# Desperodoo/distributed_multi_agent_reinforcement_learning

Hardware: AMD Instinct MI355X
Metric: env-steps/sec (whole node), pursuit-evasion 8-agent 4096-env (higher is better)
Workload: dtype f64 environment / f32 policy (f32 matrix products evaluated from exact 3-way bf16 operand splits, f32 accumulation and storage)

## Files before the change

### distributed_multi_agent_reinforcement_learning_amd/csrc/mappo_split.hip

```cpp
#include <hip/hip_runtime.h>
#include <stdint.h>
#include <string.h>

#include "mappo_ops.h"
#include "sb_gemm.hpp"
#include "sb_gru_seq.hpp"

extern "C" {

static int sb_gemm_any(int64_t R, int32_t N, int32_t K, const float *X, int64_t ldx, const float *W, int64_t ldw, const float *bias, int32_t relu,
                       const float *addend, int64_t lda, float *Y, int64_t ldy, uint8_t *ybits, int64_t ldyb, void *stream) {
    if (R < 0 || !X || !W || !Y || ldx < K || ldw < K || ldy < N || (addend && lda < N)) return MO_ERR_BAD_ARG;
    if ((ldx & 3) || (ldw & 3) || (ldy & 3) || (lda & 3) || ((uintptr_t)X & 15) || ((uintptr_t)W & 15) || ((uintptr_t)Y & 15) || ((uintptr_t)addend & 15) ||
        ((uintptr_t)bias & 15))
        return MO_ERR_BAD_ARG;
    if (R == 0) return 0;
    hipStream_t st = (hipStream_t)stream;
    if (N == 128 && K == 128) return launch_sb_gemm_best<4, 1>(R, X, ldx, W, ldw, bias, addend, lda, Y, ldy, relu, st, ybits, ldyb);
    if (N == 128 && K == 256) return launch_sb_gemm_best<8, 1>(R, X, ldx, W, ldw, bias, addend, lda, Y, ldy, relu, st, ybits, ldyb);
    if (ybits) return MO_ERR_BAD_ARG;
    if (N == 128 && K == 384) return launch_sb_gemm_best<12, 1>(R, X, ldx, W, ldw, bias, addend, lda, Y, ldy, relu, st);
    if (N == 256 && K == 128) return launch_sb_gemm_best<4, 2>(R, X, ldx, W, ldw, bias, addend, lda, Y, ldy, relu, st);
    if (N == 384 && K == 128) return launch_sb_gemm_best<4, 3>(R, X, ldx, W, ldw, bias, addend, lda, Y, ldy, relu, st);
    return MO_ERR_BAD_ARG;
}

int sb_gemm(int64_t R, int32_t N, int32_t K, const float *X, int64_t ldx, const float *W, int64_t ldw, const float *bias, int32_t relu,
            const float *addend, int64_t lda, float *Y, int64_t ldy, void *stream) {
    return sb_gemm_any(R, N, K, X, ldx, W, ldw, bias, relu, addend, lda, Y, ldy, nullptr, 0, stream);
}

int sb_gemm_signs(int64_t R, int32_t N, int32_t K, const float *X, int64_t ldx, const float *W, int64_t ldw, const float *bias, int32_t relu,
                  const float *addend, int64_t lda, float *Y, int64_t ldy, uint8_t *y_sign_bits, int64_t ld_bytes, void *stream) {
    if (!y_sign_bits || ld_bytes < N / 8) return MO_ERR_BAD_ARG;
    return sb_gemm_any(R, N, K, X, ldx, W, ldw, bias, relu, addend, lda, Y, ldy, y_sign_bits, ld_bytes, stream);
}

int64_t sb_gemm_masked_workspace(int32_t N) { return N > 0 ? (int64_t)1024 * N * 4 : 0; }

int sb_gemm_masked(int64_t R, int32_t N, int32_t K, const float *X, int64_t ldx, const float *W, int64_t ldw, const float *M, int64_t ldm,
                   int32_t mask_cols, float *Y, int64_t ldy, float *colsum, void *workspace, void *stream) {
    if (R < 0 || !X || !W || !M || !Y || !colsum || !workspace || ldx < K || ldw < K || ldy < N || ldm < N) return MO_ERR_BAD_ARG;
    if (mask_cols < 0 || mask_cols > N || (mask_cols & 127)) return MO_ERR_BAD_ARG;
    if ((ldx & 3) || (ldw & 3) || (ldy & 3) || (ldm & 3) || ((uintptr_t)X & 15) || ((uintptr_t)W & 15) || ((uintptr_t)Y & 15) || ((uintptr_t)M & 15) ||
        ((uintptr_t)colsum & 15) || ((uintptr_t)workspace & 15))
        return MO_ERR_BAD_ARG;
    hipStream_t st = (hipStream_t)stream;
    if (R == 0) return (int)hipMemsetAsync(colsum, 0, (size_t)N * 4, st);
    int dev = 0, cus = 256;
    if (hipGetDevice(&dev) == hipSuccess && hipDeviceGetAttribute(&cus, hipDeviceAttributeMultiprocessorCount, dev) != hipSuccess) cus = 256;
    if (cus > 512) return MO_ERR_BAD_ARG;
    float *part = (float *)workspace;
// ... 60 lines not shown
```

### distributed_multi_agent_reinforcement_learning_amd/csrc/sb_gemm.hpp

```cpp
#pragma once
#include <mutex>

#include "sb_common.hpp"

#ifndef SBG_ABLATE
#define SBG_ABLATE 0
#endif

template <int KC, int NT, int OPT = 3>
__global__ __launch_bounds__(512) void k_sb_gemm_n128(int64_t R, const float *__restrict__ X, int64_t ldx, const float *__restrict__ W, int64_t ldw,
                                                      const float *__restrict__ bias, const float *addend, int64_t lda, float *Y, int64_t ldy, int relu,
                                                      int mask_tiles, float *__restrict__ colsum_part, uint8_t *__restrict__ ybits = nullptr, int64_t ldyb = 0) {
    extern __shared__ uint4 sbg_tile[];
    constexpr int IMG = 3 * KC * 2 * 64, UPW = KC / 4;
    const int tid = threadIdx.x, w = tid >> 6, l = tid & 63, i = l & 15, gq = l >> 4;
    uint4 wg[NT][KC][3];
    float4 b4[NT];
#pragma unroll
    for (int t = 0; t < NT; t++) {
        const float *rw = W + (size_t)(16 * (w + 8 * t) + i) * ldw + 8 * gq;
#pragma unroll
        for (int c = 0; c < KC; c++) sb_split8(*(const float4 *)(rw + 32 * c), *(const float4 *)(rw + 32 * c + 4), wg[t][c]);
        b4[t] = !(OPT & 4) && bias ? *(const float4 *)(bias + 16 * (w + 8 * t) + 4 * gq) : make_float4(0.f, 0.f, 0.f, 0.f);
    }
    const int64_t n_it = (R + 31) / 32;
    float4 pf[UPW][2];
    auto fetch = [&](int64_t it) {
#pragma unroll
        for (int n = 0; n < UPW; n++) {
            const int blk = w * UPW + n, c = blk >> 1, rt = blk & 1;
            const int64_t row = it * 32 + rt * 16 + i;
            pf[n][0] = pf[n][1] = make_float4(0.f, 0.f, 0.f, 0.f);
            if (row < R) {
                const float *src = X + row * ldx + 32 * c + 8 * gq;
                if constexpr (SBG_ABLATE & 4) {
                    pf[n][0] = pf[n][1] = make_float4((float)row * 1e-6f, 0.5f, -0.25f, (float)c);
                } else {
                    pf[n][0] = *(const float4 *)src;
                    pf[n][1] = *(const float4 *)(src + 4);
                }
            }
        }
    };
    auto stage = [&](uint4 *img) {
#pragma unroll
        for (int n = 0; n < UPW; n++) {
            const int blk = w * UPW + n;
            uint4 p_[3];
            sb_split8(pf[n][0], pf[n][1], p_);
#pragma unroll
            for (int p = 0; p < 3; p++) img[(p * KC * 2 + blk) * 64 + l] = p_[p];
        }
    };
    int64_t it = blockIdx.x;
    if (it < n_it) { fetch(it); stage(sbg_tile); }
    if (it + gridDim.x < n_it) fetch(it + gridDim.x);
    lds_barrier();
    int cur = 0;
    float4 cs[NT];
#pragma unroll
    for (int t = 0; t < NT; t++) cs[t] = make_float4(0.f, 0.f, 0.f, 0.f);
    for (; it < n_it; it += gridDim.x) {
        const uint4 *tb = sbg_tile + cur * IMG + l;
        f32x4 acc[NT][2];
        float4 a4[NT][2];
        if ((OPT & 1) && addend) {
#pragma unroll
            for (int rt = 0; rt < 2; rt++) {
                const int64_t row = it * 32 + rt * 16 + i;
#pragma unroll
                for (int t = 0; t < NT; t++)
                    a4[t][rt] = row < R ? *(const float4 *)(addend + row * lda + 16 * (w + 8 * t) + 4 * gq) : make_float4(0.f, 0.f, 0.f, 0.f);
            }
        }
        auto next_tile = [&]() {
// ... 38 lines not shown
            if constexpr (AHEAD) __builtin_amdgcn_sched_barrier(0);
        }
        if (!(OPT & 2) || w >= 4) next_tile();
        unsigned mb[NT][2];
        if constexpr ((OPT & 4) && (OPT & 16)) {
            __builtin_amdgcn_sched_barrier(0);
            const uint8_t *bits = (const uint8_t *)addend;
#pragma unroll
            for (int rt = 0; rt < 2; rt++) {
                const int64_t row = it * 32 + rt * 16 + i;
#pragma unroll
                for (int t = 0; t < NT; t++)
                    mb[t][rt] = row < R && t < mask_tiles ? (unsigned)bits[row * lda + 2 * (w + 8 * t) + (gq >> 1)] >> ((gq & 1) * 4) : 15u;
            }
        } else if constexpr ((OPT & 4) && !(OPT & 1)) {
            __builtin_amdgcn_sched_barrier(0);
#pragma unroll
            for (int rt = 0; rt < 2; rt++) {
                const int64_t row = it * 32 + rt * 16 + i;
#pragma unroll
                for (int t = 0; t < NT; t++)
                    a4[t][rt] = row < R && t < mask_tiles ? *(const float4 *)(addend + row * lda + 16 * (w + 8 * t) + 4 * gq) : make_float4(1.f, 1.f, 1.f, 1.f);
            }
        }
#pragma unroll
        for (int rt = 0; rt < 2; rt++) {
            const int64_t row = it * 32 + rt * 16 + i;
            if (row < R) {
#pragma unroll
                for (int t = 0; t < NT; t++) {
                    const int col = 16 * (w + 8 * t) + 4 * gq;
                    float4 v;
                    if constexpr (OPT & 4) {
                        v = make_float4(acc[t][rt][0], acc[t][rt][1], acc[t][rt][2], acc[t][rt][3]);
                        if constexpr (OPT & 16) {
                            const unsigned m = mb[t][rt];
                            v.x = (m & 1u) ? v.x : 0.f; v.y = (m & 2u) ? v.y : 0.f; v.z = (m & 4u) ? v.z : 0.f; v.w = (m & 8u) ? v.w : 0.f;
                        } else if (t < mask_tiles) {
                            v.x = a4[t][rt].x > 0.f ? v.x : 0.f; v.y = a4[t][rt].y > 0.f ? v.y : 0.f;
                            v.z = a4[t][rt].z > 0.f ? v.z : 0.f; v.w = a4[t][rt].w > 0.f ? v.w : 0.f;
                        }
                        cs[t].x += v.x; cs[t].y += v.y; cs[t].z += v.z; cs[t].w += v.w;
                    } else {
                        v = make_float4(acc[t][rt][0] + b4[t].x, acc[t][rt][1] + b4[t].y, acc[t][rt][2] + b4[t].z, acc[t][rt][3] + b4[t].w);
                        if (addend) {
                            if (!(OPT & 1)) a4[t][rt] = *(const float4 *)(addend + row * lda + col);
                            v.x += a4[t][rt].x; v.y += a4[t][rt].y; v.z += a4[t][rt].z; v.w += a4[t][rt].w;
                        }
                        if (relu) { v.x = fmaxf(v.x, 0.f); v.y = fmaxf(v.y, 0.f); v.z = fmaxf(v.z, 0.f); v.w = fmaxf(v.w, 0.f); }
                        if constexpr (OPT & 8) {
                            const unsigned nib = (unsigned)(v.x > 0.f) | ((unsigned)(v.y > 0.f) << 1) | ((unsigned)(v.z > 0.f) << 2) | ((unsigned)(v.w > 0.f) << 3);
                            const unsigned other = (unsigned)__shfl_xor((int)nib, 16);
                            if (!(gq & 1)) ybits[row * ldyb + 2 * (w + 8 * t) + (gq >> 1)] = (uint8_t)(nib | (other << 4));
                        }
                    }
                    if constexpr (SBG_ABLATE & 2) { if (v.x == 12345.678f) *(float4 *)(Y + row * ldy + col) = v; }
                    else *(float4 *)(Y + row * ldy + col) = v;
                }
            }
        }
        lds_barrier();
        cur ^= 1;
    }
    if constexpr (OPT & 4) {
#pragma unroll
        for (int t = 0; t < NT; t++) {
#pragma unroll
            for (int m = 1; m < 16; m <<= 1) {
                cs[t].x += __shfl_xor(cs[t].x, m); cs[t].y += __shfl_xor(cs[t].y, m);
                cs[t].z += __shfl_xor(cs[t].z, m); cs[t].w += __shfl_xor(cs[t].w, m);
            }
            if (i == 0) *(float4 *)(colsum_part + (size_t)blockIdx.x * (128 * NT) + 16 * (w + 8 * t) + 4 * gq) = cs[t];
        }
    }
}

__global__ void k_sb_colsum_reduce(int n_parts, int F, const float *__restrict__ parts, float *__restrict__ out) {
    const int f = blockIdx.x * blockDim.x + threadIdx.x;
    if (f >= F) return;
    float a0 = 0.f, a1 = 0.f, a2 = 0.f, a3 = 0.f;
    int p = 0;
    for (; p + 4 <= n_parts; p += 4) {
        a0 += parts[(size_t)p * F + f]; a1 += parts[(size_t)(p + 1) * F + f];
        a2 += parts[(size_t)(p + 2) * F + f]; a3 += parts[(size_t)(p + 3) * F + f];
    }
    for (; p < n_parts; p++) a0 += parts[(size_t)p * F + f];
    out[f] = (a0 + a1) + (a2 + a3);
}

static int g_sbg_wgs_per_cu = 0;

template <int KC, int NT, int OPT>
int launch_sb_gemm(int64_t R, const float *X, int64_t ldx, const float *W, int64_t ldw, const float *bias, const float *addend, int64_t lda,
                   float *Y, int64_t ldy, int relu, hipStream_t st, int mask_tiles = 0, float *colsum_part = nullptr, float *colsum = nullptr,
                   uint8_t *ybits = nullptr, int64_t ldyb = 0) {
    constexpr int lds = 2 * 3 * KC * 2 * 64 * 16;
    static std::once_flag once;
    static hipError_t attr_rc = hipSuccess;
    std::call_once(once, [] { attr_rc = hipFuncSetAttribute((const void *)k_sb_gemm_n128<KC, NT, OPT>, hipFuncAttributeMaxDynamicSharedMemorySize, lds); });
    if (attr_rc != hipSuccess) return (int)attr_rc;
    int dev = 0, cus = 256;
    if (hipGetDevice(&dev) == hipSuccess && hipDeviceGetAttribute(&cus, hipDeviceAttributeMultiprocessorCount, dev) != hipSuccess) cus = 256;
    const int64_t n_it = (R + 31) / 32;
    const int wpc = g_sbg_wgs_per_cu ? g_sbg_wgs_per_cu : (KC * NT == 4 && R >= 131072 ? 2 : 1);
    const int grid = n_it < (int64_t)cus * wpc ? (int)n_it : cus * wpc;
    hipLaunchKernelGGL((k_sb_gemm_n128<KC, NT, OPT>), dim3(grid), dim3(512), lds, st, R, X, ldx, W, ldw, bias, addend, lda, Y, ldy, relu, mask_tiles,
                       colsum_part, ybits, ldyb);
    if constexpr (OPT & 4) hipLaunchKernelGGL(k_sb_colsum_reduce, dim3((128 * NT + 127) / 128), dim3(128), 0, st, grid, 128 * NT, colsum_part, colsum);
    return (int)hipGetLastError();
}

constexpr int SBG_MASK_OPT_256 = 6, SBG_MASK_OPT_384 = 4, SBG_MASK_OPT_K384 = 6;

template <int KC, int NT>
int launch_sb_gemm_best(int64_t R, const float *X, int64_t ldx, const float *W, int64_t ldw, const float *bias, const float *addend, int64_t lda,
                        float *Y, int64_t ldy, int relu, hipStream_t st, uint8_t *ybits = nullptr, int64_t ldyb = 0) {
    constexpr int PLAIN = (KC == 4 && NT == 1) ? 0 : 2;
    constexpr int ADD = KC == 12 ? 2 : (KC == 8 ? 3 : (NT == 3 ? 0 : 1));
    if constexpr (NT == 1 && KC <= 8) if (ybits) {
        if (addend) return launch_sb_gemm<KC, NT, ADD | 8>(R, X, ldx, W, ldw, bias, addend, lda, Y, ldy, relu, st, 0, nullptr, nullptr, ybits, ldyb);
        if constexpr (KC == 4 && NT == 1) if (R >= 786432) return launch_sb_gemm<4, 1, 10>(R, X, ldx, W, ldw, bias, addend, lda, Y, ldy, relu, st, 0, nullptr, nullptr, ybits, ldyb);
        return launch_sb_gemm<KC, NT, PLAIN | 8>(R, X, ldx, W, ldw, bias, addend, lda, Y, ldy, relu, st, 0, nullptr, nullptr, ybits, ldyb);
    }
    if (addend) return launch_sb_gemm<KC, NT, ADD>(R, X, ldx, W, ldw, bias, addend, lda, Y, ldy, relu, st);
    if constexpr (KC == 4 && NT == 1) if (R >= 786432) return launch_sb_gemm<4, 1, 2>(R, X, ldx, W, ldw, bias, addend, lda, Y, ldy, relu, st);
    return launch_sb_gemm<KC, NT, PLAIN>(R, X, ldx, W, ldw, bias, addend, lda, Y, ldy, relu, st);
}
```

### distributed_multi_agent_reinforcement_learning_amd/model.py

```python
import torch
import torch.nn as nn
import torch.nn.functional as F
from torch.nn.utils import spectral_norm
from torch.nn.utils.spectral_norm import SpectralNorm

from . import ops


class HeadLinear(nn.Linear):

    def forward(self, x):
        return ops.linear_skinny(x, self.weight, self.bias)


def _ortho_linear(n_in, n_out, cls=nn.Linear):
    layer = cls(n_in, n_out)
    for name, param in layer.named_parameters():
        if "bias" in name:
            nn.init.constant_(param, 0)
        elif "weight" in name:
            nn.init.orthogonal_(param, gain=1.0)
    return layer


# ... 26 lines not shown
        self.AGG_layers["AGG_vertex_0"] = _make_linear(E, E, is_sn)
        for k in range(self.depth):
            self.AGG_layers[f"AGG_fcra_{k}"] = _make_linear(E, E, is_sn)

    def encoder(self, p, e, o, adj_p, adj_e, adj_o, is_critic, o_kvalid=None, q_div=1, out=None, e_ref=None):
        M = self.MSG_layers
        m3 = ops.msg_agg3(p, e, o, adj_p, adj_e, adj_o, M[0].weight, M[0].bias, M[1].weight, M[1].bias, M[2].weight, M[2].bias,
                          is_critic, o_kvalid, q_div, e_ref)
        return self._after_messages(p, m3, out)

    def _after_messages(self, p, m3, out=None):
        R, P = p.shape[0], p.shape[1]
        E, ind = self.embedding_dim, self.input_dim
        agg0 = self.AGG_layers["AGG_vertex_0"]
        link = ops.ReluLink()
        emb = ops.linear(m3, agg0.weight, agg0.bias, relu=True, y_link=link)
        Ws = self.semantic_layer.weight
        p2, e2 = p.reshape(R * P, ind), emb.reshape(R * P, 3 * E)
        if out is not None:
            o2 = out.view(R * P, E)
            torch.addmm(self.semantic_layer.bias, p2, Ws[:, :ind].t(), out=o2)
            h0 = o2.addmm_(e2, Ws[:, ind:].t())
        else:
            h0 = ops.linear(e2, Ws[:, ind:], ops.linear_skinny(p2, Ws[:, :ind], self.semantic_layer.bias), consume_addend=True, x_link=link)
        return h0.reshape(R, P, E)

    def encoder_pair_train(self, p, e, o, adj_p, adj_e, adj_o, q_div=1, e_ref=None):
        M = self.MSG_layers
        m3a, m3c = ops.msg_agg3_pair_train(p, e, o, adj_p, adj_e, adj_o, M[0].weight, M[0].bias, M[1].weight, M[1].bias, M[2].weight, M[2].bias,
                                           q_div, e_ref)
        return self._after_messages(p, m3a), self._after_messages(p, m3c)

    def fcra(self, h0, hist, adj_p, is_critic, out=None):
        if self.depth == 0:
            return h0
        h, carry = h0, None
        for k in range(self.depth):
            aggk, fk = self.AGG_layers[f"AGG_fcra_{k}"], self.FCRA_layers[k]
            nb = ops.fcra_mean(z_critic=hist[k]) if is_critic else ops.fcra_mean(z_actor=hist[k], adj=adj_p)
            last = k == self.depth - 1
            h, carry = ops.fcra_hop(nb, h, carry, aggk.weight, aggk.bias, fk.weight, fk.bias, last, out if last else None)
        h.relu_link = carry[1]
        return h

    def forward(self, p, e, o, adj_p, adj_e, adj_o, hist, is_critic, o_kvalid=None, q_div=1, out=None, e_ref=None):
        h0 = self.encoder(p, e, o, adj_p, adj_e, adj_o, is_critic, o_kvalid, q_div, out if self.depth == 0 else None, e_ref)
        return self.fcra(h0, hist, adj_p, is_critic, out)

    def forward_pair(self, p, e, o, adj_p, adj_e, adj_o, hist_a, hist_c, o_kvalid=None, q_div=1, out=None, e_ref=None):
        R, P = p.shape[0], p.shape[1]
        E, ind = self.embedding_dim, self.input_dim
        M = self.MSG_layers
        Ws = self.semantic_layer.weight
        d = self.depth
        cats = [torch.empty((2, R, P, 2 * E), dtype=p.dtype, device=p.device) for _ in range(d)]
        if d:
            h0 = cats[0][..., E:]
        else:
            h0 = out if out is not None else torch.empty((2, R, P, E), dtype=p.dtype, device=p.device)
        h0_2d = ops.block2d(h0)
        fused_pos = ind == 4
        m3 = ops.msg_agg3_pair(p, e, o, adj_p, adj_e, adj_o, M[0].weight, M[0].bias, M[1].weight, M[1].bias, M[2].weight, M[2].bias,
                               o_kvalid, q_div, pos=(Ws[:, :ind], self.semantic_layer.bias, h0) if fused_pos else None, e_ref=e_ref)
        agg0 = self.AGG_layers["AGG_vertex_0"]
        m3_2d = m3.view(-1, E)
        if ops.split_linear_ok(m3_2d, agg0.weight):
            emb = ops.split_linear(m3_2d, agg0.weight, agg0.bias, relu=True).view(m3.shape)
        else:
            emb = ops.linear(m3, agg0.weight, agg0.bias, relu=True)
        if not fused_pos:
            torch.addmm(self.semantic_layer.bias, p.reshape(R * P, ind), Ws[:, :ind].t(), out=h0_2d[:R * P])
            h0_2d[R * P:].copy_(h0_2d[:R * P])
        emb_2d, Wse = emb.view(2 * R * P, 3 * E), Ws[:, ind:]
        if ops.split_linear_ok(emb_2d, Wse, h0_2d, h0_2d):
            ops.split_linear(emb_2d, Wse, None, False, out=h0_2d, addend=h0_2d)
        elif d:
            ops.gemm_nt(emb_2d, Wse, None, False, out=h0_2d, addend=h0_2d)
        else:
            h0_2d.addmm_(emb_2d, Wse.t())
        if d == 0:
            return h0
        h = h0
        zas, zcs = [], []
        for k in range(d):
            aggk = self.AGG_layers[f"AGG_fcra_{k}"]

            def lin(z, W=aggk.weight):
                if z.is_contiguous() and ops.split_linear_ok(z.view(-1, E), W):
                    return ops.split_linear(z.view(-1, E), W).view(z.shape)
                return ops.linear(z, W)
            za = lin(hist_a[k])
            zcs.append(za if hist_c[k] is hist_a[k] or hist_c[k].data_ptr() == hist_a[k].data_ptr() else lin(hist_c[k]))
            zas.append(za)
        if d <= 4 and all(z.is_contiguous() for z in zas + zcs) and adj_p.dtype == torch.float32:
            ops.fcra_mean_pair_multi(zas, zcs, adj_p, [self.AGG_layers[f"AGG_fcra_{k}"].bias for k in range(d)], [cats[k][..., :E] for k in range(d)])
        else:
            for k in range(d):
# ... 233 lines not shown
```

### distributed_multi_agent_reinforcement_learning_amd/ops.py

```python
import ctypes as C
import os

import torch
import torch.nn.functional as F

from . import build as _build

ADJ_TENSOR, ADJ_ONES, ADJ_VALID, ADJ_BITS = 0, 1, 2, 3
EXPORTS = ("dhgn_msg_agg_fwd", "dhgn_msg_agg3_fwd", "dhgn_msg_agg_bwd", "dhgn_msg_agg_bwd_workspace", "dhgn_msg_agg_ones_sorted_ok", "dhgn_msg_agg_ones_sorted_fwd",
           "dhgn_msg_agg_ones_sorted_bwd", "dhgn_msg_agg_ones_sorted_workspace", "gae_advnorm", "gae_advnorm_workspace", "categorical_sample",
           "categorical_sample_counter",
           "gru_gates_fwd", "gru_gates_bwd", "gru_cell_fwd", "gru_cell_fwd_multi", "gru_cell_split_fwd_multi", "sb_gemm_n128", "sb_gemm", "gru_seq_fwd", "gru_seq_fwd_multi", "gru_seq_split_fwd_multi", "gru_seq_split_bwd_multi", "gru_seq_save_elems", "gru_seq_bwd", "gru_seq_bwd_multi", "gru_seq_bwd_workspace", "wgrad_tn", "wgrad_tn_workspace", "wgrad_split_tn", "wgrad_split_tn2", "wgrad_split_workspace", "rollout_record", "ppo_loss_fwd_bwd", "ppo_loss_prob_fwd_bwd", "ppo_loss_workspace",
           "gauss_head_sample", "ppo_loss_gauss_fwd_bwd", "ppo_loss_gauss_workspace", "gauss_head_sample_ex", "ppo_loss_gauss_ex_fwd_bwd",
           "ppo_loss_gauss_ex_workspace", "gae_advnorm_vn", "gae_advnorm_vn_workspace", "value_norm_update", "value_norm_targets",
           "ppo_loss_fwd_bwd_diag", "ppo_loss_prob_fwd_bwd_diag", "ppo_loss_gauss_fwd_bwd_diag", "ppo_loss_gauss_ex_fwd_bwd_diag",
           "ppo_loss_diag_workspace", "ppo_loss_gauss_diag_workspace", "ppo_ratio", "ppo_diag_rows_host", "fused_adam_workspace",
           "fused_adam_grid", "fused_adam_norm", "fused_adam_step", "fused_adam_advance_host", "fused_adam_rows_host", "bc_loss_workspace",
           "bc_loss_gauss_fwd_bwd", "bc_loss_gauss_ex_fwd_bwd", "bc_loss_cat_fwd_bwd", "e3d_bc_select", "n2n_bc_select", "mappo_ops_error_string")

_lib = None


def lib_path():
    return _build.lib_path("libmappo_ops.so")


def load_library():
    global _lib
    if _lib is None:
        path = lib_path()
        if not os.path.exists(path):
            raise RuntimeError(f"{path} is missing: build it with __graft_entry__.build() (hipcc --offload-arch=gfx950); "
                               "the fused MAPPO ops have no fallback")
        L = C.CDLL(path)
        vp, i32, i64, f32, f64 = C.c_void_p, C.c_int32, C.c_int64, C.c_float, C.c_double
# ... 11 lines not shown
        L.dhgn_msg_agg_ones_sorted_workspace.argtypes = [i32, i32, i32, i32, i32, vp, vp, vp]
        L.dhgn_msg_agg_ones_sorted_workspace.restype = i64
        L.dhgn_msg_agg_ones_sorted_fwd.argtypes = [i32, i32, i32, i32, vp, i64, vp, i64, i32, vp, vp, vp, i64, vp, vp, vp]
        L.dhgn_msg_agg_ones_sorted_bwd.argtypes = [i32, i32, i32, i32, vp, i64, i32, vp, i64, vp, vp, vp, vp, vp, vp]
        L.gae_advnorm.argtypes = [i32, i32, i32, vp, vp, vp, f32, f32, i32, vp, vp, vp, vp]
        L.gae_advnorm_workspace.restype = i64
        L.gae_advnorm_vn.argtypes = [i32, i32, i32, vp, vp, vp, vp, vp, f32, f32, i32, vp, vp, vp, vp, vp]
        L.gae_advnorm_vn_workspace.restype = i64
        L.value_norm_update.argtypes = [vp, vp, C.c_double, vp]
        L.value_norm_targets.argtypes = [i64, vp, vp, vp, vp, vp]
        L.categorical_sample.argtypes = [i32, i32, vp, C.c_uint64, C.c_uint64, i32, vp, vp, vp]
        L.categorical_sample_counter.argtypes = [i32, i32, vp, C.c_uint64, vp, i32, vp, vp, vp]
        L.head_linear.argtypes = [i32, i32, i32, vp, vp, vp, vp, vp]
        L.head_sample.argtypes = [i32, i32, i32, vp, vp, vp, C.c_uint64, vp, vp, i32, vp, vp, vp]
        L.gru_gates_fwd.argtypes = [i32, i32, vp, vp, vp, vp, vp, vp, vp]
        L.gru_gates_bwd.argtypes = [i32, i32, vp, vp, vp, vp, vp, vp, vp, vp]
        L.gru_cell_fwd.argtypes = [i32, i32, vp, vp, vp, vp, vp, vp, vp, vp]
        L.gru_seq_fwd.argtypes = [i32, i32, i32, vp, vp, vp, vp, vp, vp, i32, vp]
        L.gru_seq_bwd.argtypes = [i32, i32, i32, vp, vp, vp, vp, vp, vp, vp, vp, vp, vp, vp, i32, vp, vp]
        L.gru_cell_fwd_multi.argtypes = [i32, vp, i32, i32, vp]
        L.gru_cell_split_fwd_multi.argtypes = [i32, vp, i32, i32, vp]
        L.sb_gemm_n128.argtypes = [i64, i32, vp, i64, vp, i64, vp, i32, vp, i64, vp, i64, vp]
        L.sb_gemm.argtypes = [i64, i32, i32, vp, i64, vp, i64, vp, i32, vp, i64, vp, i64, vp]
        L.gru_seq_fwd_multi.argtypes = [i32, vp, i32, i32, i32, i32, vp]
        L.gru_seq_bwd_multi.argtypes = [i32, vp, i32, i32, i32, i32, vp]
        L.gru_seq_split_fwd_multi.argtypes = [i32, vp, i32, i32, i32, i32, vp]
        L.gru_seq_split_bwd_multi.argtypes = [i32, vp, i32, i32, i32, i32, vp]
        L.gru_seq_save_elems.argtypes = [i32, i32]
        L.gru_seq_save_elems.restype = i64
        L.gru_seq_bwd_workspace.argtypes = [i32]
        L.gru_seq_bwd_workspace.restype = i64
        L.wgrad_tn_workspace.argtypes = [i32, i32]
        L.wgrad_tn_workspace.restype = i64
        L.wgrad_tn.argtypes = [i64, i32, i32, vp, i64, vp, i64, vp, i32, vp, vp]
        L.wgrad_split_workspace.restype = i64
        L.wgrad_split_workspace.argtypes = [i32, i32]
        L.wgrad_split_tn.argtypes = [i64, i32, i32, vp, i64, vp, i64, vp, i32, vp, vp]
        L.wgrad_split_tn2.argtypes = [i64, i32, i32, i32, vp, i64, vp, i64, vp, i64, vp, i32, vp, vp]
        L.fcra_neighbour_mean.argtypes = [i32, i32, i32, i32, vp, i64, i64, vp, i64, i64, vp, i64, vp, i32, vp, vp, i64, vp]
        L.fcra_neighbour_mean_multi.argtypes = [i32, vp, i32, i32, i32, i32, i64, i64, i64, i64, vp, i64, i32, i64, vp]
        L.sb_gemm_signs.argtypes = [i64, i32, i32, vp, i64, vp, i64, vp, i32, vp, i64, vp, i64, vp, i64, vp]
        L.sb_gemm_masked_bits.argtypes = [i64, i32, i32, vp, i64, vp, i64, vp, i64, i32, vp, i64, vp, vp, vp]
        L.sb_gemm_masked_workspace.argtypes = [i32]
        L.sb_gemm_masked_workspace.restype = i64
        L.sb_gemm_masked.argtypes = [i64, i32, i32, vp, i64, vp, i64, vp, i64, i32, vp, i64, vp, vp, vp]
        L.relu_bwd_colsum_workspace.argtypes = [i32]
# ... 1552 lines not shown
    MATMUL_MODE, WGRAD_MODE, PROJ_MODE, CELL_MODE, SEQ_MODE = modes


def set_matmul_mode(mode):
    global MATMUL_MODE, WGRAD_MODE, PROJ_MODE, SEQ_MODE
    set_cell_mode(mode)
    MATMUL_MODE = WGRAD_MODE = PROJ_MODE = SEQ_MODE = mode


SPLIT_LINEAR_SHAPES = {(128, 128), (128, 256), (128, 384), (256, 128), (384, 128)}
UPDATE_SPLIT_SHAPES = SPLIT_LINEAR_SHAPES


def split_linear_ok(x, W, out=None, addend=None, mode=None, shapes=None):
    if ((CELL_MODE if mode is None else mode) != "split_bf16" or torch.is_grad_enabled() or not x.is_cuda
            or tuple(W.shape) not in (SPLIT_LINEAR_SHAPES if shapes is None else shapes)):
        return False
    for t in (x, W) + ((out,) if out is not None else ()) + ((addend,) if addend is not None else ()):
        if t.dtype != torch.float32 or t.dim() != 2 or t.stride(1) != 1 or t.stride(0) % 4 or t.data_ptr() % 16:
            return False
    return x.shape[1] == W.shape[1]


def split_linear(x, W, bias=None, relu=False, out=None, addend=None, sign_bits=None):
    L = load_library()
    R, K = x.shape
    N = W.shape[0]
    W = W.detach()
    if out is None:
        out = torch.empty((R, N), dtype=torch.float32, device=x.device)
    b = bias.detach() if bias is not None else None
    if sign_bits is not None:
        assert sign_bits.dtype == torch.uint8 and sign_bits.shape == (R, N // 8) and sign_bits.stride(1) == 1 and sign_bits_ok(N, K)
        _check(L.sb_gemm_signs(R, N, K, _ptr(x), x.stride(0), _ptr(W), W.stride(0), _ptr(b), int(bool(relu)), _ptr(addend),
                               addend.stride(0) if addend is not None else 0, _ptr(out), out.stride(0), _ptr(sign_bits), sign_bits.stride(0), _stream()),
               "sb_gemm_signs")
        return out
    _check(L.sb_gemm(R, N, K, _ptr(x), x.stride(0), _ptr(W), W.stride(0), _ptr(b), int(bool(relu)), _ptr(addend),
                     addend.stride(0) if addend is not None else 0, _ptr(out), out.stride(0), _stream()), "sb_gemm")
    return out


def sign_bits_ok(N, K):
    return RELU_LINK and RELU_BITS and N == 128 and K in (128, 256)


PROJ_MODE = os.environ.get("MAPPO_PROJ", MATMUL_MODE)


def gru_input_projection(x2, w_ih, b_ih):
    if x2.stride(-1) == 1 and split_linear_ok(x2, w_ih, mode=PROJ_MODE, shapes=UPDATE_SPLIT_SHAPES):
        return split_linear(x2, w_ih, b_ih)
    return torch.addmm(b_ih, x2, w_ih.t())


def gru_step_multi(xs, hiddens, modules, hiddens_out=None):
    n = len(xs)
    B = xs[0].shape[0]
    outs_h = hiddens if hiddens_out is None else hiddens_out
    ok = (not torch.is_grad_enabled() and n <= 4 and B >= FUSED_CELL_MIN_ROWS and all(x.shape == (B, 128) and x.is_cuda for x in xs)
          and all(h.is_contiguous() and h.shape[1:] == (B, 128) for h in list(hiddens) + list(outs_h))
          and all(m.num_layers == modules[0].num_layers and m.weight_hh_l0.shape == (384, 128) and m.weight_ih_l0.shape == (384, 128) for m in modules))
    if not ok:
# ... 203 lines not shown
```

### include/mappo_ops.h

```cpp
#ifndef MAPPO_OPS_H
#define MAPPO_OPS_H
#include <stdint.h>

#ifdef __cplusplus
extern "C" {
#endif

#define MO_ERR_BAD_ARG 20001

enum { MO_ADJ_TENSOR = 0,
       MO_ADJ_ONES = 1,
       MO_ADJ_VALID = 2,
       MO_ADJ_BITS = 3 };
#define MO_ADJ_ROW_WORDS(K) (((((K) + 31) >> 5) + 3) & ~3)

int dhgn_msg_agg_fwd(int32_t R, int32_t P, int32_t K, int32_t E, int32_t din, const float *p, int64_t p_row_stride,
                     const float *q, int64_t q_row_stride, int32_t q_div, const float *e, int64_t e_row_stride, const void *adj,
                     int64_t adj_row_stride, int32_t adj_mode, const int32_t *kvalid, const float *W, const float *b,
                     float *out, int64_t out_stride , void *stream);

typedef struct mo_msg_rel {
    int32_t K, din, q_div, adj_mode;
    const float *q; int64_t q_rs;
    const float *e; int64_t e_rs;
// ... 79 lines not shown
    void *workspace;
    int32_t B, pad0;
} mo_gru_seq_bwd_net;
int gru_seq_fwd_multi(int32_t n_nets, const mo_gru_seq_net *nets, int32_t T, int32_t B, int32_t H, int32_t gi_agents, void *stream);
int gru_seq_bwd_multi(int32_t n_nets, const mo_gru_seq_bwd_net *nets, int32_t T, int32_t B, int32_t H, int32_t gi_agents, void *stream);
int gru_seq_split_fwd_multi(int32_t n_nets, const mo_gru_seq_net *nets, int32_t T, int32_t B, int32_t H, int32_t gi_agents, void *stream);
int gru_seq_split_bwd_multi(int32_t n_nets, const mo_gru_seq_bwd_net *nets, int32_t T, int32_t B, int32_t H, int32_t gi_agents, void *stream);
int gru_seq_fwd(int32_t T, int32_t B, int32_t H, const float *gi, const float *w_hh, const float *b_hh, const float *h0, float *out,
                float *save, int32_t gi_agents, void *stream);
int64_t gru_seq_bwd_workspace(int32_t B);
int gru_seq_bwd(int32_t T, int32_t B, int32_t H, const float *dout, const float *save, const float *out, const float *h0,
                const float *w_hh, float *dgi, float *dgh, float *dnr, float *dh0, float *db_ih, float *db_hh, int32_t gi_agents,
                void *workspace, void *stream);

int gru_cell_fwd(int32_t B, int32_t H, const float *x, const float *h_prev, const float *w_ih, const float *w_hh, const float *b_ih,
                 const float *b_hh, float *h_out, void *stream);
typedef struct mo_gru_cell_net { const float *x, *h_prev, *w_ih, *w_hh, *b_ih, *b_hh; float *h_out; } mo_gru_cell_net;
int gru_cell_fwd_multi(int32_t n_nets, const mo_gru_cell_net *nets, int32_t B, int32_t H, void *stream);
int gru_cell_split_fwd_multi(int32_t n_nets, const mo_gru_cell_net *nets, int32_t B, int32_t H, void *stream);
int sb_gemm_n128(int64_t R, int32_t K, const float *X, int64_t ldx, const float *W, int64_t ldw, const float *bias, int32_t relu, const float *C,
                 int64_t ldc, float *Y, int64_t ldy, void *stream);
int sb_gemm(int64_t R, int32_t N, int32_t K, const float *X, int64_t ldx, const float *W, int64_t ldw, const float *bias, int32_t relu, const float *C,
            int64_t ldc, float *Y, int64_t ldy, void *stream);
int sb_gemm_signs(int64_t R, int32_t N, int32_t K, const float *X, int64_t ldx, const float *W, int64_t ldw, const float *bias, int32_t relu, const float *C,
                  int64_t ldc, float *Y, int64_t ldy, uint8_t *y_sign_bits, int64_t ld_bytes, void *stream);
int64_t sb_gemm_masked_workspace(int32_t N);
int sb_gemm_masked(int64_t R, int32_t N, int32_t K, const float *X, int64_t ldx, const float *W, int64_t ldw, const float *M, int64_t ldm,
                   int32_t mask_cols, float *Y, int64_t ldy, float *colsum, void *workspace, void *stream);
int sb_gemm_masked_bits(int64_t R, int32_t N, int32_t K, const float *X, int64_t ldx, const float *W, int64_t ldw, const uint8_t *sign_bits,
                        int64_t ld_bytes, int32_t mask_cols, float *Y, int64_t ldy, float *colsum, void *workspace, void *stream);

int64_t ppo_loss_workspace(void);
int ppo_loss_fwd_bwd(int64_t n, const float *logp_now, const float *entropy, const float *logp_old, const float *adv, const float *active,
                     const float *values_now, const float *values_old, const float *v_target, const float *active_sum, float epsilon,
                     float entropy_coef, int32_t use_value_clip, float *losses, float *grad_logp, float *grad_entropy, float *grad_values,
                     void *workspace, void *stream);
int ppo_loss_prob_fwd_bwd(int64_t n, int32_t A, const float *prob, float *grad_prob, int64_t d1, int64_t d2, int64_t p_s0, int64_t p_s1, int64_t p_s2,
                          const float *action, const float *logp_old, const float *adv, const float *active, const float *values_now, int64_t v_s0,
                          int64_t v_s1, int64_t v_s2, const float *values_old, const float *v_target, const float *active_sum, float epsilon,
                          float entropy_coef, int32_t use_value_clip, float *losses, float *grad_values, void *workspace, void *stream);

int gauss_head_sample(int32_t R, int32_t A, int32_t H, const float *feat, const float *W, const float *b, const float *log_std, uint64_t seed,
                      uint64_t *counter, uint32_t *ticket, int32_t greedy, float *action, double *env_action, float *logp, void *stream);
int64_t ppo_loss_gauss_workspace(void);
int ppo_loss_gauss_fwd_bwd(int64_t n, int32_t A, const float *mu, float *grad_mu, int64_t d1, int64_t d2, int64_t m_s0, int64_t m_s1, int64_t m_s2,
                           const float *log_std, const float *action, const float *logp_old, const float *adv, const float *active,
// ... 103 lines not shown
```

Before: 2.650 million.

## Fuse 4-wide position projection into semantic GEMM epilogue

Adds a position-epilogue variant of the split-bf16 128x384 GEMM that computes the skinny K=4 position projection plus bias inside the epilogue. This replaces the separate addend pass, where h0 was written by the message-aggregation kernel or a skinny linear and then read back as an addend. The position rows are staged in LDS alongside the X tiles, and row wrap handles the duplicated pair halves. The default mode 'rollout' enables it only for no-grad rollout encoder_pair calls. Training uses it only when the env var is set to 1, and that path carries a new autograd function with its own backward. It adds LDS usage and epilogue FMAs.

```diff
diff --git a/distributed_multi_agent_reinforcement_learning_amd/csrc/mappo_split.hip b/distributed_multi_agent_reinforcement_learning_amd/csrc/mappo_split.hip
--- a/distributed_multi_agent_reinforcement_learning_amd/csrc/mappo_split.hip
+++ b/distributed_multi_agent_reinforcement_learning_amd/csrc/mappo_split.hip
@@ -28,6 +28,20 @@
 int sb_gemm(int64_t R, int32_t N, int32_t K, const float *X, int64_t ldx, const float *W, int64_t ldw, const float *bias, int32_t relu,
             const float *addend, int64_t lda, float *Y, int64_t ldy, void *stream) {
     return sb_gemm_any(R, N, K, X, ldx, W, ldw, bias, relu, addend, lda, Y, ldy, nullptr, 0, stream);
+}
+
+int sb_gemm_pos(int64_t R, int32_t N, int32_t K, const float *X, int64_t ldx, const float *W, int64_t ldw, const float *bias, int32_t relu,
+                const float *p, int64_t ldp, int64_t p_rows, const float *Wp, int64_t ldwp, const float *bp, float *Y, int64_t ldy, void *stream) {
+    if (N != 128 || K != 384) return MO_ERR_BAD_ARG;
+    if (R < 0 || !X || !W || !Y || !p || !Wp || !bp || ldx < K || ldw < K || ldy < N || ldp < 4 || ldwp < 4) return MO_ERR_BAD_ARG;
+    if (p_rows < 1 || R > 2 * p_rows) return MO_ERR_BAD_ARG;
+    if (ldx >= (1 << 24) || ldy >= (1 << 24) || ldp >= (1 << 24)) return MO_ERR_BAD_ARG;
+    if ((ldx & 3) || (ldw & 3) || (ldy & 3) || ((uintptr_t)X & 15) || ((uintptr_t)W & 15) || ((uintptr_t)Y & 15) || ((uintptr_t)bias & 15) ||
+        ((uintptr_t)p & 3) || ((uintptr_t)Wp & 3) || ((uintptr_t)bp & 3))
+        return MO_ERR_BAD_ARG;
+    if (R == 0) return 0;
+    return launch_sb_gemm<12, 1, SBG_POS_OPT>(R, X, ldx, W, ldw, bias, nullptr, 0, Y, ldy, relu, (hipStream_t)stream, 0, nullptr, nullptr, nullptr, 0,
+                                              SbgPos{p, ldp, p_rows, Wp, ldwp, bp});
 }
 
 int sb_gemm_signs(int64_t R, int32_t N, int32_t K, const float *X, int64_t ldx, const float *W, int64_t ldw, const float *bias, int32_t relu,
diff --git a/distributed_multi_agent_reinforcement_learning_amd/csrc/sb_gemm.hpp b/distributed_multi_agent_reinforcement_learning_amd/csrc/sb_gemm.hpp
--- a/distributed_multi_agent_reinforcement_learning_amd/csrc/sb_gemm.hpp
+++ b/distributed_multi_agent_reinforcement_learning_amd/csrc/sb_gemm.hpp
@@ -7,13 +7,37 @@
 #define SBG_ABLATE 0
 #endif
 
+struct SbgPos {
+    const float *p;
+    int64_t ldp, p_rows;
+    const float *Wp;
+    int64_t ldwp;
+    const float *bp;
+};
+constexpr int SBG_POS_LDS = (6 * 128 + 2 * 128) * 4;
+
 template <int KC, int NT, int OPT = 3>
 __global__ __launch_bounds__(512) void k_sb_gemm_n128(int64_t R, const float *__restrict__ X, int64_t ldx, const float *__restrict__ W, int64_t ldw,
                                                       const float *__restrict__ bias, const float *addend, int64_t lda, float *Y, int64_t ldy, int relu,
-                                                      int mask_tiles, float *__restrict__ colsum_part, uint8_t *__restrict__ ybits = nullptr, int64_t ldyb = 0) {
+                                                      int mask_tiles, float *__restrict__ colsum_part, uint8_t *__restrict__ ybits = nullptr, int64_t ldyb = 0,
+                                                      SbgPos pos = SbgPos{}) {
     extern __shared__ uint4 sbg_tile[];
     constexpr int IMG = 3 * KC * 2 * 64, UPW = KC / 4;
+    static_assert(!(OPT & 32) || (KC == 12 && NT == 1 && !(OPT & (1 | 4 | 8 | 16))), "the position epilogue: 128 <- 384, no addend, mask or sign bits");
     const int tid = threadIdx.x, w = tid >> 6, l = tid & 63, i = l & 15, gq = l >> 4;
+    float *const pos_tab = (float *)(sbg_tile + 2 * IMG), *const pos_rows = pos_tab + 6 * 128;
+    float pp = 0.f;
+    const int ws = __builtin_amdgcn_readfirstlane(w);
+    const unsigned xoff = (unsigned)(i * (int)ldx + 8 * gq) * 4u, yoff = (unsigned)(i * (int)ldy + 4 * gq) * 4u;
+    const unsigned poff = (unsigned)((tid >> 2) * (int)pos.ldp + (tid & 3)) * 4u;
+    if constexpr (OPT & 32) {
+        if (tid < 128) {
+#pragma unroll
+            for (int k = 0; k < 4; k++) pos_tab[k * 128 + tid] = pos.Wp[(size_t)tid * pos.ldwp + k];
+            pos_tab[4 * 128 + tid] = pos.bp[tid];
+            pos_tab[5 * 128 + tid] = bias ? bias[tid] : 0.f;
+        }
+    }
     uint4 wg[NT][KC][3];
     float4 b4[NT];
 #pragma unroll
@@ -21,11 +45,29 @@
         const float *rw = W + (size_t)(16 * (w + 8 * t) + i) * ldw + 8 * gq;
 #pragma unroll
         for (int c = 0; c < KC; c++) sb_split8(*(const float4 *)(rw + 32 * c), *(const float4 *)(rw + 32 * c + 4), wg[t][c]);
-        b4[t] = !(OPT & 4) && bias ? *(const float4 *)(bias + 16 * (w + 8 * t) + 4 * gq) : make_float4(0.f, 0.f, 0.f, 0.f);
+        b4[t] = !(OPT & (4 | 32)) && bias ? *(const float4 *)(bias + 16 * (w + 8 * t) + 4 * gq) : make_float4(0.f, 0.f, 0.f, 0.f);
     }
     const int64_t n_it = (R + 31) / 32;
     float4 pf[UPW][2];
     auto fetch = [&](int64_t it) {
+        if constexpr (OPT & 32) {
+            const int live = R - it * 32 < 32 ? (int)(R - it * 32) : 32;
+            const char *xb = (const char *)(X + it * 32 * ldx);
+#pragma unroll
+            for (int n = 0; n < UPW; n++) {
+                const int blk = ws * UPW + n, c = blk >> 1, rt = blk & 1;
+                pf[n][0] = pf[n][1] = make_float4(0.f, 0.f, 0.f, 0.f);
+                if (rt * 16 + i < live) {
+                    const char *src = xb + ((int64_t)rt * 16 * ldx + 32 * c) * 4;
+                    pf[n][0] = *(const float4 *)(src + xoff);
+                    pf[n][1] = *(const float4 *)(src + xoff + 16);
+                }
+            }
+            const int64_t wrap = it * 32 + (tid >> 2) < pos.p_rows ? 0 : pos.p_rows;
+            pp = 0.f;
+            if (tid < 128 && (tid >> 2) < live) pp = *(const float *)((const char *)pos.p + ((it * 32 - wrap) * pos.ldp * 4 + (int64_t)poff));
+            return;
+        }
 #pragma unroll
         for (int n = 0; n < UPW; n++) {
             const int blk = w * UPW + n, c = blk >> 1, rt = blk & 1;
@@ -51,6 +93,9 @@
 #pragma unroll
             for (int p = 0; p < 3; p++) img[(p * KC * 2 + blk) * 64 + l] = p_[p];
         }
+        if constexpr (OPT & 32) {
+            if (tid < 128) pos_rows[(img == sbg_tile ? 0 : 128) + tid] = pp;
+        }
     };
     int64_t it = blockIdx.x;
     if (it < n_it) { fetch(it); stage(sbg_tile); }
@@ -135,6 +180,13 @@
                 for (int t = 0; t < NT; t++)
                     a4[t][rt] = row < R && t < mask_tiles ? *(const float4 *)(addend + row * lda + 16 * (w + 8 * t) + 4 * gq) : make_float4(1.f, 1.f, 1.f, 1.f);
             }
+        }
+        float4 pt[5];
+        if constexpr (OPT & 32) {
+            __builtin_amdgcn_sched_barrier(0);
+#pragma unroll
+            for (int k = 0; k < 5; k++) pt[k] = *(const float4 *)(pos_tab + k * 128 + 16 * w + 4 * gq);
+            b4[0] = *(const float4 *)(pos_tab + 5 * 128 + 16 * w + 4 * gq);
         }
 #pragma unroll
         for (int rt = 0; rt < 2; rt++) {
@@ -156,9 +208,16 @@
                         cs[t].x += v.x; cs[t].y += v.y; cs[t].z += v.z; cs[t].w += v.w;
                     } else {
                         v = make_float4(acc[t][rt][0] + b4[t].x, acc[t][rt][1] + b4[t].y, acc[t][rt][2] + b4[t].z, acc[t][rt][3] + b4[t].w);
-                        if (addend) {
+                        if (!(OPT & 32) && addend) {
                             if (!(OPT & 1)) a4[t][rt] = *(const float4 *)(addend + row * lda + col);
                             v.x += a4[t][rt].x; v.y += a4[t][rt].y; v.z += a4[t][rt].z; v.w += a4[t][rt].w;
+                        }
+                        if constexpr (OPT & 32) {
+                            const float4 q = *(const float4 *)(pos_rows + cur * 128 + (rt * 16 + i) * 4);
+                            v.x += __builtin_fmaf(pt[3].x, q.w, __builtin_fmaf(pt[2].x, q.z, __builtin_fmaf(pt[1].x, q.y, __builtin_fmaf(pt[0].x, q.x, pt[4].x))));
+                            v.y += __builtin_fmaf(pt[3].y, q.w, __builtin_fmaf(pt[2].y, q.z, __builtin_fmaf(pt[1].y, q.y, __builtin_fmaf(pt[0].y, q.x, pt[4].y))));
+                            v.z += __builtin_fmaf(pt[3].z, q.w, __builtin_fmaf(pt[2].z, q.z, __builtin_fmaf(pt[1].z, q.y, __builtin_fmaf(pt[0].z, q.x, pt[4].z))));
+                            v.w += __builtin_fmaf(pt[3].w, q.w, __builtin_fmaf(pt[2].w, q.z, __builtin_fmaf(pt[1].w, q.y, __builtin_fmaf(pt[0].w, q.x, pt[4].w))));
                         }
                         if (relu) { v.x = fmaxf(v.x, 0.f); v.y = fmaxf(v.y, 0.f); v.z = fmaxf(v.z, 0.f); v.w = fmaxf(v.w, 0.f); }
                         if constexpr (OPT & 8) {
@@ -168,6 +227,7 @@
                         }
                     }
                     if constexpr (SBG_ABLATE & 2) { if (v.x == 12345.678f) *(float4 *)(Y + row * ldy + col) = v; }
+                    else if constexpr (OPT & 32) *(float4 *)((char *)(Y + (it * 32 + rt * 16) * ldy + 16 * ws) + yoff) = v;
                     else *(float4 *)(Y + row * ldy + col) = v;
                 }
             }
@@ -206,8 +266,8 @@
 template <int KC, int NT, int OPT>
 int launch_sb_gemm(int64_t R, const float *X, int64_t ldx, const float *W, int64_t ldw, const float *bias, const float *addend, int64_t lda,
                    float *Y, int64_t ldy, int relu, hipStream_t st, int mask_tiles = 0, float *colsum_part = nullptr, float *colsum = nullptr,
-                   uint8_t *ybits = nullptr, int64_t ldyb = 0) {
-    constexpr int lds = 2 * 3 * KC * 2 * 64 * 16;
+                   uint8_t *ybits = nullptr, int64_t ldyb = 0, SbgPos pos = SbgPos{}) {
+    constexpr int lds = 2 * 3 * KC * 2 * 64 * 16 + ((OPT & 32) ? SBG_POS_LDS : 0);
     static std::once_flag once;
     static hipError_t attr_rc = hipSuccess;
     std::call_once(once, [] { attr_rc = hipFuncSetAttribute((const void *)k_sb_gemm_n128<KC, NT, OPT>, hipFuncAttributeMaxDynamicSharedMemorySize, lds); });
@@ -218,11 +278,12 @@
     const int wpc = g_sbg_wgs_per_cu ? g_sbg_wgs_per_cu : (KC * NT == 4 && R >= 131072 ? 2 : 1);
     const int grid = n_it < (int64_t)cus * wpc ? (int)n_it : cus * wpc;
     hipLaunchKernelGGL((k_sb_gemm_n128<KC, NT, OPT>), dim3(grid), dim3(512), lds, st, R, X, ldx, W, ldw, bias, addend, lda, Y, ldy, relu, mask_tiles,
-                       colsum_part, ybits, ldyb);
+                       colsum_part, ybits, ldyb, pos);
     if constexpr (OPT & 4) hipLaunchKernelGGL(k_sb_colsum_reduce, dim3((128 * NT + 127) / 128), dim3(128), 0, st, grid, 128 * NT, colsum_part, colsum);
     return (int)hipGetLastError();
 }
 
+constexpr int SBG_POS_OPT = 2 | 32;
 constexpr int SBG_MASK_OPT_256 = 6, SBG_MASK_OPT_384 = 4, SBG_MASK_OPT_K384 = 6;
 
 template <int KC, int NT>
diff --git a/distributed_multi_agent_reinforcement_learning_amd/model.py b/distributed_multi_agent_reinforcement_learning_amd/model.py
--- a/distributed_multi_agent_reinforcement_learning_amd/model.py
+++ b/distributed_multi_agent_reinforcement_learning_amd/model.py
@@ -72,7 +72,9 @@
             torch.addmm(self.semantic_layer.bias, p2, Ws[:, :ind].t(), out=o2)
             h0 = o2.addmm_(e2, Ws[:, ind:].t())
         else:
-            h0 = ops.linear(e2, Ws[:, ind:], ops.linear_skinny(p2, Ws[:, :ind], self.semantic_layer.bias), consume_addend=True, x_link=link)
+            h0 = ops.semantic_linear(e2, Ws[:, ind:], p2, Ws[:, :ind], self.semantic_layer.bias, link) if ind == 4 else None
+            if h0 is None:
+                h0 = ops.linear(e2, Ws[:, ind:], ops.linear_skinny(p2, Ws[:, :ind], self.semantic_layer.bias), consume_addend=True, x_link=link)
         return h0.reshape(R, P, E)
 
     def encoder_pair_train(self, p, e, o, adj_p, adj_e, adj_o, q_div=1, e_ref=None):
@@ -110,8 +112,12 @@
             h0 = out if out is not None else torch.empty((2, R, P, E), dtype=p.dtype, device=p.device)
         h0_2d = ops.block2d(h0)
         fused_pos = ind == 4
+        Wse = Ws[:, ind:]
+        p2 = p.reshape(R * P, ind) if p.stride(2) == 1 and p.stride(0) == P * p.stride(1) else None
+        epi_pos = (fused_pos and p2 is not None and ops.POS_EPILOGUE != "0" and ops.CELL_MODE == "split_bf16" and not torch.is_grad_enabled()
+                   and ops.pos_epilogue_ok(None, Wse, p2, Ws[:, :ind], 2 * R * P, h0_2d))
         m3 = ops.msg_agg3_pair(p, e, o, adj_p, adj_e, adj_o, M[0].weight, M[0].bias, M[1].weight, M[1].bias, M[2].weight, M[2].bias,
-                               o_kvalid, q_div, pos=(Ws[:, :ind], self.semantic_layer.bias, h0) if fused_pos else None, e_ref=e_ref)
+                               o_kvalid, q_div, pos=(Ws[:, :ind], self.semantic_layer.bias, h0) if fused_pos and not epi_pos else None, e_ref=e_ref)
         agg0 = self.AGG_layers["AGG_vertex_0"]
         m3_2d = m3.view(-1, E)
         if ops.split_linear_ok(m3_2d, agg0.weight):
@@ -121,8 +127,10 @@
         if not fused_pos:
             torch.addmm(self.semantic_layer.bias, p.reshape(R * P, ind), Ws[:, :ind].t(), out=h0_2d[:R * P])
             h0_2d[R * P:].copy_(h0_2d[:R * P])
-        emb_2d, Wse = emb.view(2 * R * P, 3 * E), Ws[:, ind:]
-        if ops.split_linear_ok(emb_2d, Wse, h0_2d, h0_2d):
+        emb_2d = emb.view(2 * R * P, 3 * E)
+        if epi_pos:
+            ops.split_linear(emb_2d, Wse, None, False, out=h0_2d, pos=(p2, Ws[:, :ind], self.semantic_layer.bias))
+        elif ops.split_linear_ok(emb_2d, Wse, h0_2d, h0_2d):
             ops.split_linear(emb_2d, Wse, None, False, out=h0_2d, addend=h0_2d)
         elif d:
             ops.gemm_nt(emb_2d, Wse, None, False, out=h0_2d, addend=h0_2d)
diff --git a/distributed_multi_agent_reinforcement_learning_amd/ops.py b/distributed_multi_agent_reinforcement_learning_amd/ops.py
--- a/distributed_multi_agent_reinforcement_learning_amd/ops.py
+++ b/distributed_multi_agent_reinforcement_learning_amd/ops.py
@@ -10,7 +10,7 @@
 EXPORTS = ("dhgn_msg_agg_fwd", "dhgn_msg_agg3_fwd", "dhgn_msg_agg_bwd", "dhgn_msg_agg_bwd_workspace", "dhgn_msg_agg_ones_sorted_ok", "dhgn_msg_agg_ones_sorted_fwd",
            "dhgn_msg_agg_ones_sorted_bwd", "dhgn_msg_agg_ones_sorted_workspace", "gae_advnorm", "gae_advnorm_workspace", "categorical_sample",
            "categorical_sample_counter",
-           "gru_gates_fwd", "gru_gates_bwd", "gru_cell_fwd", "gru_cell_fwd_multi", "gru_cell_split_fwd_multi", "sb_gemm_n128", "sb_gemm", "gru_seq_fwd", "gru_seq_fwd_multi", "gru_seq_split_fwd_multi", "gru_seq_split_bwd_multi", "gru_seq_save_elems", "gru_seq_bwd", "gru_seq_bwd_multi", "gru_seq_bwd_workspace", "wgrad_tn", "wgrad_tn_workspace", "wgrad_split_tn", "wgrad_split_tn2", "wgrad_split_workspace", "rollout_record", "ppo_loss_fwd_bwd", "ppo_loss_prob_fwd_bwd", "ppo_loss_workspace",
+           "gru_gates_fwd", "gru_gates_bwd", "gru_cell_fwd", "gru_cell_fwd_multi", "gru_cell_split_fwd_multi", "sb_gemm_n128", "sb_gemm", "sb_gemm_pos", "gru_seq_fwd", "gru_seq_fwd_multi", "gru_seq_split_fwd_multi", "gru_seq_split_bwd_multi", "gru_seq_save_elems", "gru_seq_bwd", "gru_seq_bwd_multi", "gru_seq_bwd_workspace", "wgrad_tn", "wgrad_tn_workspace", "wgrad_split_tn", "wgrad_split_tn2", "wgrad_split_workspace", "rollout_record", "ppo_loss_fwd_bwd", "ppo_loss_prob_fwd_bwd", "ppo_loss_workspace",
            "gauss_head_sample", "ppo_loss_gauss_fwd_bwd", "ppo_loss_gauss_workspace", "gauss_head_sample_ex", "ppo_loss_gauss_ex_fwd_bwd",
            "ppo_loss_gauss_ex_workspace", "gae_advnorm_vn", "gae_advnorm_vn_workspace", "value_norm_update", "value_norm_targets",
            "ppo_loss_fwd_bwd_diag", "ppo_loss_prob_fwd_bwd_diag", "ppo_loss_gauss_fwd_bwd_diag", "ppo_loss_gauss_ex_fwd_bwd_diag",
@@ -68,6 +68,7 @@
         L.gru_cell_split_fwd_multi.argtypes = [i32, vp, i32, i32, vp]
         L.sb_gemm_n128.argtypes = [i64, i32, vp, i64, vp, i64, vp, i32, vp, i64, vp, i64, vp]
         L.sb_gemm.argtypes = [i64, i32, i32, vp, i64, vp, i64, vp, i32, vp, i64, vp, i64, vp]
+        L.sb_gemm_pos.argtypes = [i64, i32, i32, vp, i64, vp, i64, vp, i32, vp, i64, i64, vp, i64, vp, vp, i64, vp]
         L.gru_seq_fwd_multi.argtypes = [i32, vp, i32, i32, i32, i32, vp]
         L.gru_seq_bwd_multi.argtypes = [i32, vp, i32, i32, i32, i32, vp]
         L.gru_seq_split_fwd_multi.argtypes = [i32, vp, i32, i32, i32, i32, vp]
@@ -1666,7 +1667,7 @@
     return x.shape[1] == W.shape[1]
 
 
-def split_linear(x, W, bias=None, relu=False, out=None, addend=None, sign_bits=None):
+def split_linear(x, W, bias=None, relu=False, out=None, addend=None, sign_bits=None, pos=None):
     L = load_library()
     R, K = x.shape
     N = W.shape[0]
@@ -1674,6 +1675,13 @@
     if out is None:
         out = torch.empty((R, N), dtype=torch.float32, device=x.device)
     b = bias.detach() if bias is not None else None
+    if pos is not None:
+        p2, Wp, bp = pos
+        Wp, bp = Wp.detach(), bp.detach().contiguous()
+        assert addend is None and sign_bits is None and pos_epilogue_ok(x, W, p2, Wp, R, out)
+        _check(L.sb_gemm_pos(R, N, K, _ptr(x), x.stride(0), _ptr(W), W.stride(0), _ptr(b), int(bool(relu)), _ptr(p2), p2.stride(0), p2.shape[0],
+                             _ptr(Wp), Wp.stride(0), _ptr(bp), _ptr(out), out.stride(0), _stream()), "sb_gemm_pos")
+        return out
     if sign_bits is not None:
         assert sign_bits.dtype == torch.uint8 and sign_bits.shape == (R, N // 8) and sign_bits.stride(1) == 1 and sign_bits_ok(N, K)
         _check(L.sb_gemm_signs(R, N, K, _ptr(x), x.stride(0), _ptr(W), W.stride(0), _ptr(b), int(bool(relu)), _ptr(addend),
@@ -1683,6 +1691,62 @@
     _check(L.sb_gemm(R, N, K, _ptr(x), x.stride(0), _ptr(W), W.stride(0), _ptr(b), int(bool(relu)), _ptr(addend),
                      addend.stride(0) if addend is not None else 0, _ptr(out), out.stride(0), _stream()), "sb_gemm")
     return out
+
+
+POS_EPILOGUE = os.environ.get("MAPPO_POS_EPILOGUE", "rollout")
+if POS_EPILOGUE not in ("0", "rollout", "1"):
+    raise ValueError(f"MAPPO_POS_EPILOGUE={POS_EPILOGUE!r}: 0 | rollout | 1")
+
+
+def pos_epilogue_ok(x, W, p2, Wp, rows, out=None):
+    if not W.is_cuda or tuple(W.shape) != (128, 384) or (x is not None and tuple(x.shape) != (rows, 384)) or p2.dim() != 2 or p2.shape[1] != 4:
+        return False
+    if p2.shape[0] != rows and 2 * p2.shape[0] != rows:
+        return False
+    for t in (W,) + ((x,) if x is not None else ()) + ((out,) if out is not None else ()):
+        if t.dtype != torch.float32 or t.dim() != 2 or t.stride(1) != 1 or t.stride(0) % 4 or t.data_ptr() % 16 or t.stride(0) >= 1 << 24:
+            return False
+    return (p2.dtype == torch.float32 and Wp.dtype == torch.float32 and tuple(Wp.shape) == (128, 4) and p2.stride(1) == 1 and Wp.stride(1) == 1
+            and 4 <= p2.stride(0) < 1 << 24 and Wp.stride(0) >= 4)
+
+
+class _SemanticLinear(torch.autograd.Function):
+
+    @staticmethod
+    def forward(ctx, e2, W, p2, Wp, bp, x_link):
+        ctx.x_link = x_link
+        ctx.save_for_backward(e2, W, p2, Wp)
+        return split_linear(e2, W, pos=(p2, Wp, bp))
+
+    @staticmethod
+    def backward(ctx, g):
+        e2, W, p2, Wp = ctx.saved_tensors
+        g2 = g if g.stride(1) == 1 else g.contiguous()
+        dx = None
+        if ctx.needs_input_grad[0]:
+            fused = None
+            if ctx.x_link is not None:
+                bits = ctx.x_link.bits
+                fused = input_grad_masked(g2, W, e2, W.shape[1], bits.view(e2.shape[0], -1) if bits is not None else None)
+            if fused is not None:
+                dx, ctx.x_link.db = fused
+            else:
+                dx = input_grad(g2, W)
+        dW = wgrad(g2, e2) if ctx.needs_input_grad[1] else None
+        dp = torch.mm(g2, Wp) if ctx.needs_input_grad[2] else None
+        dWp = dbp = None
+        if ctx.needs_input_grad[3] or ctx.needs_input_grad[4]:
+            dWp, dbp, _ = wgrad_skinny(p2, g2, transposed=True, colsum_x=ctx.needs_input_grad[4])
+        return dx, dW, dp, dWp, dbp, None
+
+
+def semantic_linear(e2, W, p2, Wp, bp, x_link=None):
+    if (POS_EPILOGUE != "1" or PROJ_MODE != "split_bf16" or not e2.is_cuda or e2.stride(-1) != 1 or not e2.shape[0]
+            or not pos_epilogue_ok(e2, W, p2, Wp, e2.shape[0]) or p2.shape[0] != e2.shape[0]):
+        return None
+    if torch.is_grad_enabled() and any(t.requires_grad for t in (e2, W, p2, Wp, bp)):
+        return _SemanticLinear.apply(e2, W, p2, Wp, bp, x_link)
+    return split_linear(e2, W, pos=(p2, Wp, bp))
 
 
 def sign_bits_ok(N, K):
diff --git a/include/mappo_ops.h b/include/mappo_ops.h
--- a/include/mappo_ops.h
+++ b/include/mappo_ops.h
@@ -125,6 +125,8 @@
                  int64_t ldc, float *Y, int64_t ldy, void *stream);
 int sb_gemm(int64_t R, int32_t N, int32_t K, const float *X, int64_t ldx, const float *W, int64_t ldw, const float *bias, int32_t relu, const float *C,
             int64_t ldc, float *Y, int64_t ldy, void *stream);
+int sb_gemm_pos(int64_t R, int32_t N, int32_t K, const float *X, int64_t ldx, const float *W, int64_t ldw, const float *bias, int32_t relu,
+                const float *p, int64_t ldp, int64_t p_rows, const float *Wp, int64_t ldwp, const float *bp, float *Y, int64_t ldy, void *stream);
 int sb_gemm_signs(int64_t R, int32_t N, int32_t K, const float *X, int64_t ldx, const float *W, int64_t ldw, const float *bias, int32_t relu, const float *C,
                   int64_t ldc, float *Y, int64_t ldy, uint8_t *y_sign_bits, int64_t ld_bytes, void *stream);
 int64_t sb_gemm_masked_workspace(int32_t N);
```

New measurement: 2.676 million (median of 6 runs). No clear change (+1.0%).
